# grospy/bitcoincashplus

Measured on AMD Instinct MI355X. Metric: equihash_200_9_solutions_per_sec, higher is better.
Workload: dtype uint32; 1 GPU; model=Equihash(200,9) mainnet PoW solver (BLAKE2b, K=9 collision rounds), global_batch=96, seq_len=2097152, parallelism=dp1 (nonce-space), solvers_in_flight=2, full=False, verified_solutions=0, gpu_cpu_verifier_disagreements=0, rows_dropped_all_nonces=232040, pairs_dropped_all_nonces=346057, candidates_dropped_all_nonces=0

## Files before the change

csrc/kernels/equihash_layout.h:

```cpp
#ifndef BCP_KERNELS_EQUIHASH_LAYOUT_H
#define BCP_KERNELS_EQUIHASH_LAYOUT_H

#include <cstddef>
#include <cstdint>
#include <stdexcept>

#if defined(__HIPCC__)
#define BCP_EH_HD __host__ __device__
#else
#define BCP_EH_HD
#endif

#ifndef BCP_EH_GEN_HPT
#define BCP_EH_GEN_HPT 2
#endif
#ifndef BCP_EH_GEN_NT
#define BCP_EH_GEN_NT 512
#endif
#ifndef BCP_EH_PRUNE_FROM
#define BCP_EH_PRUNE_FROM 9
#endif
#ifndef BCP_EH_MP_LATE
#define BCP_EH_MP_LATE 1
#endif
#ifndef BCP_EH_MP_LATE_FROM
#define BCP_EH_MP_LATE_FROM 8
#endif
#ifndef BCP_EH_GW
#define BCP_EH_GW 4
#endif
#ifndef BCP_EH_TABLE_PARENTS
#define BCP_EH_TABLE_PARENTS 1
#endif

namespace bcpk {

template <class C> constexpr int round_nt(int stage, bool carry);
template <class C> constexpr int round_mp(int stage, bool carry = false);
template <class C> constexpr bool round_prunes(int stage, bool carry = false);

template <int N_, int K_, int BB_, int CAP_, int NT_, int GENWG_, int NTG_, int MAXCAND_, int CAP4_ = CAP_,
          int CAP3_ = CAP_, int WGCU_ = 1, int GNT_ = 512, int GHPT_ = 2, int CAPF_ = 0, int MPX_ = 0, int GW_ = 0>
struct EhCfg {
    static constexpr int N = N_, K = K_;
    static constexpr int DB = N / (K + 1);
    static constexpr int BB = BB_;
    static constexpr int RB = DB - BB_;
    static constexpr int NB = 1 << BB_;
    static constexpr int NRESTS = 1 << RB;
    static constexpr int CAP = CAP_;
    static constexpr int CAPF = CAPF_ > 0 ? CAPF_ : CAP3_;
    static constexpr int MPX = MPX_;
    static constexpr int cap(int round) {
        return round == K_ ? CAPF : words(round - 1) >= 5 ? CAP_ : words(round - 1) == 4 ? CAP4_ : CAP3_;
// ... 32 lines not shown
    static constexpr bool tp(int stage) {
        return BCP_EH_TABLE_PARENTS && stage >= 1 && stage <= K - 2 && !round_prunes<EhCfg>(stage + 1) &&
               !round_prunes<EhCfg>(stage + 1, true) && pad(stage) >= BB;
    }
    static constexpr int ptab(int stage) {
        const int a = round_mp<EhCfg>(stage, false) * round_nt<EhCfg>(stage, false);
        const int b = GW_ > 0 ? round_mp<EhCfg>(stage, true) * round_nt<EhCfg>(stage, true) : 0;
        return a > b ? a : b;
    }
    static constexpr uint32_t tpmask(int stage) { return (1u << (pad(stage) > BB ? BB + 1 : BB)) - 1; }
    static constexpr uint32_t rmask(int stage) { return tp(stage) ? (uint32_t)NB - 1 : cp(stage) ? RMASK : 0u; }
    static constexpr int sw(int stage) {
        return stage == 0 || tp(stage) ? words(stage) : words(stage) + (cp(stage) ? 1 : 2);
    }
    static constexpr size_t ROWS = (size_t)NB * AREA;
    static constexpr bool H16 = NB > 512;
    static constexpr int HW = H16 ? NB / 2 : NB;
    static_assert(RPW * GENWG_ == INIT && RPW < 65535, "generation split");
    static_assert(RB > 0 && DB < 32, "digit geometry");
    static_assert(AREA < (1 << IB), "LDS row indices in parent words and signatures");
    static_assert(NT_ % 64 == 0 && NT_ <= 1024 && (NB <= NT_ || NB % NT_ == 0) && NB <= NTG_ && NT_ / 64 <= 64,
                  "workgroup shape");
    static_assert(words(K - 1) == 1, "final round keeps whole rows in one LDS word");
    static_assert(GW_ == 0 || (WGCU_ == 1 && RNT >= 128 && (NB <= RNT || NB % RNT == 0)), "carrying workgroup shape");
};

#ifndef BCP_EH_CAPF
#define BCP_EH_CAPF 6016
#endif
using Cfg200_9 = EhCfg<200, 9, 9, 4416, 1024, 512, 1024, 256, 4864, 5120, 1, BCP_EH_GEN_NT, BCP_EH_GEN_HPT, BCP_EH_CAPF, 0, BCP_EH_GW>;
// ... 33 lines not shown
    if (stage == C::K) return un_walk_list<C>(cap);
    const int pairs = round_mp<C>(stage, carry) * round_nt<C>(stage, carry) * 4;
    const int walk = un_walk_list<C>(cap) + pairs;
    return walk > pairs ? walk : pairs;
}
template <class C> constexpr int round_lds(int stage, bool prune, bool carry = false) {
    const int WR = C::words(stage - 1);
    const int WI = WR;
    const int cap = C::cap(stage);
    const int pruneb = prune ? cap * 4 + (C::cp(stage - 1) ? 0 : (cap * 2 + 3) / 4 * 4) : 0;
    const int hists = stage == C::K ? 0 : 2 * C::HW * 4 + (C::NB * (C::H16 ? 2 : 4) + 3) / 4 * 4;
    const int gen = carry ? 2 * C::NB * 4 + 16 * 8 : 0;
    return (cap * WI + 3) / 4 * 16 + pruneb + 4 + round_un<C>(stage, carry) + hists +
           (round_nt<C>(stage, carry) / 64 + 1) * 4 + gen;
}
template <class C> constexpr bool round_prunes(int stage, bool carry) {
    constexpr int from = C::K == 9 ? BCP_EH_PRUNE_FROM : 2;
    return (stage >= from || stage == C::K) && stage >= 2 && round_lds<C>(stage, true, carry) <= C::LDS_BUDGET;
}

template <class C> struct GenCarry {
    static constexpr int GT = C::GW > 0 ? 64 * C::GW : 64;
    static constexpr int NHASH = (C::INIT + C::IPH - 1) / C::IPH;
    static constexpr int ITERS = (C::K - 1) * C::NB;
    static constexpr int HB = ((NHASH + ITERS - 1) / ITERS + GT - 1) / GT;
    static constexpr int CH = HB * GT;
    static constexpr int RPT = HB * C::IPH;
    static constexpr int BPT = (C::NB + GT - 1) / GT;
    static_assert((long long)CH * ITERS >= NHASH, "the carrying rounds cover every hash");
};

template <class C> BCP_EH_HD inline uint64_t slot_parent(int stage, const uint32_t* slot) {
    const uint32_t* q = slot + C::words(stage);
// ... 29 lines not shown
```

csrc/kernels/equihash_solver.hip:

```cpp
#include <hip/hip_runtime.h>

#include "crypto/hashes.h"
#include "kernels/blake2b_device.h"
#include "kernels/equihash_layout.h"
#include "kernels/equihash_pow.h"
#include "kernels/gpu_api.h"
#include "kernels/hip_util.h"

#include <algorithm>
#include <cstdlib>
#include <cstring>
#include <stdexcept>
#include <utility>

#ifndef BCP_EH_XCD_MAP
#define BCP_EH_XCD_MAP 1
#endif
#ifndef BCP_EH_PF_SLICES
#define BCP_EH_PF_SLICES 3
#endif
#ifndef BCP_EH_GROUPS_DEFAULT
#define BCP_EH_GROUPS_DEFAULT(batch) ((batch) >= 48 ? (batch) / 24 : 1)
#endif

namespace bcpk {

constexpr uint32_t OOB = 0x80000000u;
typedef uint32_t u2v __attribute__((ext_vector_type(2)));
typedef uint32_t u3v __attribute__((ext_vector_type(3)));
typedef uint32_t u4v __attribute__((ext_vector_type(4)));

template <int CTRL, int ROWMASK = 0xf>
__device__ __forceinline__ uint32_t dpp0(uint32_t x) {
    return (uint32_t)__builtin_amdgcn_update_dpp(0, (int)x, CTRL, ROWMASK, 0xf, false);
// ... 308 lines not shown
#define EH_STAMP(k)                                                                                  \
    do {                                                                                             \
        if constexpr (STAMP) {                                                                       \
            if (threadIdx.x == 0) stamps[(size_t)bk * 16 + (k)] = __builtin_amdgcn_s_memtime();        \
        }                                                                                            \
    } while (0)

struct EhCarry {
    const EhBaseState* states;
    uint32_t* R0;
    uint32_t* LEAF;
    uint32_t* CTR0;
    int nonces;
};

constexpr int EH_NBAR = 10;
constexpr int EH_SCAN_BARS = 2;
template <int K> __device__ __forceinline__ void eh_bar() {
    static_assert(K >= 1 && K <= EH_NBAR, "barrier outside the bucket iteration's count");
    __syncthreads();
}
#define EH_BAR_SCAN(k) static_assert((k) >= 1 && (k) + EH_SCAN_BARS - 1 <= EH_NBAR, "scan barriers")

template <class C, int STAGE>
__device__ __forceinline__ void eh_carry_gen(const EhCarry& cy, int nbk, uint32_t* ghist, uint32_t* gbase, uint64_t* gr0p) {
    using GC = GenCarry<C>;
    constexpr int W0 = C::words(0);
    constexpr int SW = (C::N + 31) / 32 + 1;
    constexpr int SW0 = C::sw(0);
    constexpr int GT = GC::GT, HB = GC::HB;
    constexpr uint32_t OCAP = C::cap(1);
    const int gtid = (int)threadIdx.x - C::RNT;
    const int G = gridDim.x;
    auto chunk_of = [&](int b) -> int {
        const int nonce = b / C::NB, c = (STAGE - 1) * C::NB + b % C::NB;
        return (nonce < cy.nonces && (long long)c * GC::CH < GC::NHASH) ? c : -1;
    };
    auto prefix = [&](int b) {
        if (gtid == 0 && b / C::NB < cy.nonces) {
            uint64_t P[16];
            eh_hdr_round0_uniform(cy.states[b / C::NB], P);
#pragma unroll
            for (int i = 0; i < 16; ++i) gr0p[i] = P[i];
        }
    };
    constexpr int RA = 3, RB = 5, RC = 6, RD = 10;
    EhHdrHash hs[HB];
    auto start = [&](int b) {
        const int c = chunk_of(b);
        if (c < 0) return;
        const EhBaseState& bs = cy.states[b / C::NB];
        uint64_t P[16];
#pragma unroll
        for (int i = 0; i < 16; ++i) P[i] = gr0p[i];
#pragma unroll
        for (int hh = 0; hh < HB; ++hh) {
            hs[hh].begin(P, bs, (uint32_t)c * GC::CH + (uint32_t)(hh * GT + gtid));
            hs[hh].template rounds<1, RA>(bs);
        }
    };
    int it = 0;
// ... 5 lines not shown
    for (;;) {
        const int nonce = bk / C::NB;
        const int chunk = chunk_of(bk);
        const bool act = chunk >= 0;
        const EhBaseState& bs = cy.states[act ? nonce : 0];
        const int bn = xcd_bucket<C::NB>(blockIdx.x, it + 1, G, nbk);
        const bool more = bn >= 0;
        const uint32_t g0 = (uint32_t)chunk * GC::CH + (uint32_t)gtid;
        uint32_t rw[GC::RPT][W0];
        uint32_t rk[GC::RPT];
        uint32_t myb[GC::BPT];
        if (act) {
#pragma unroll
            for (int hh = 0; hh < HB; ++hh) hs[hh].template rounds<RA, RB>(bs);
        }
        eh_bar<1>();
        eh_bar<2>();
        eh_bar<3>();
        if (act) {
#pragma unroll
            for (int hh = 0; hh < HB; ++hh) hs[hh].template rounds<RB, RC>(bs);
        }
        eh_bar<4>();
        if (act) {
#pragma unroll
            for (int hh = 0; hh < HB; ++hh) hs[hh].template rounds<RC, RD>(bs);
        }
        if (more && bn / C::NB != nonce) prefix(bn);
        eh_bar<5>();
        if (act) {
#pragma unroll
            for (int hh = 0; hh < HB; ++hh) {
                hs[hh].template rounds<RD, 12>(bs);
                uint64_t h[8];
                hs[hh].finish(bs, h);
                const uint32_t g = g0 + hh * GT;
#pragma unroll
                for (int s = 0; s < C::IPH; ++s) {
                    uint32_t S[SW];
#pragma unroll
                    for (int w = 0; w < SW; ++w) {
                        uint32_t v = 0;
#pragma unroll
                        for (int t = 0; t < 4; ++t) {
                            const int k = 4 * w + t;
                            v = (v << 8) | ((k < C::NBYTES) ? digest_byte(h, s * C::NBYTES + k) : 0u);
                        }
                        S[w] = v;
                    }
                    const int q = hh * C::IPH + s;
                    const uint32_t d = S[0] >> (32 - C::BB);
#pragma unroll
                    for (int w = 0; w < W0; ++w) rw[q][w] = (S[w] << C::BB) | (S[w + 1] >> (32 - C::BB));
                    rk[q] = NIL;
                    if (g * C::IPH + s < (uint32_t)C::INIT) rk[q] = (atomicAdd(&ghist[d], 1u) << 16) | d;
                }
            }
        }
        eh_bar<6>();
        if (act) {
#pragma unroll
            for (int k = 0; k < GC::BPT; ++k) {
                const int b = gtid + k * GT;
                const uint32_t c = b < C::NB ? ghist[b] : 0u;
                myb[k] = 0;
                if (c) myb[k] = atomicAdd(&cy.CTR0[(size_t)nonce * C::NB + b], c);
            }
        }
        eh_bar<7>();
        if (act)
            for (int i = gtid; i < C::NB; i += GT) ghist[i] = 0;
        eh_bar<8>();
        if (act) {
#pragma unroll
            for (int k = 0; k < GC::BPT; ++k) {
                const int b = gtid + k * GT;
                if (b < C::NB) gbase[b] = myb[k];
            }
        }
        eh_bar<9>();
        if (act) {
            const auto rs = buf_rsrc(cy.R0 + (size_t)nonce * C::ROWS * SW0, (uint32_t)(C::ROWS * SW0 * 4));
            const auto rl = buf_rsrc(cy.LEAF + (size_t)nonce * C::ROWS, (uint32_t)(C::ROWS * 4));
#pragma unroll
            for (int q = 0; q < GC::RPT; ++q) {
                const uint32_t d = rk[q] & 0xffff;
                const uint32_t pos = gbase[d < (uint32_t)C::NB ? d : 0] + (rk[q] >> 16);
                const uint32_t slot = d * C::AREA + pos;
                const bool ok = rk[q] != NIL && pos < OCAP;
                const uint32_t li = (g0 + (q / C::IPH) * GT) * C::IPH + (q % C::IPH);
                row_store<W0>(rs, ok ? slot * (SW0 * 4) : OOB, rw[q]);
                __builtin_amdgcn_raw_buffer_store_b32(li, rl, ok ? slot * 4 : OOB, 0, 0);
            }
        }
        if (more) start(bn);
        eh_bar<EH_NBAR>();
        if (!more) break;
        bk = bn;
        ++it;
    }
}

template <class C, int STAGE, bool STAMP, bool CARRY = false>
__global__ __launch_bounds__(C::NT) __attribute__((amdgpu_waves_per_eu(C::WGCU * C::NT / 256)))
void eh_round(const uint32_t* __restrict__ Rin, const uint32_t* __restrict__ CTRin, uint32_t* __restrict__ Rout,
              uint32_t* __restrict__ CTRout, uint32_t* __restrict__ Pout, uint32_t* __restrict__ Bout,
              uint32_t* __restrict__ ncand, uint64_t* __restrict__ cand, uint64_t* __restrict__ stamps,
              uint32_t* __restrict__ pdrop, int nbk, EhCarry carry) {
    constexpr int WI = C::words(STAGE - 1);
    constexpr int WO = (STAGE < C::K) ? C::words(STAGE) : 1;
    constexpr int CAP = C::cap(STAGE);
    constexpr bool FINAL = STAGE == C::K;
    constexpr int PDW = 2 * C::K + 2;
    static_assert(!CARRY || (C::GW > 0 && !FINAL && !STAMP), "only plain collision rounds carry generation");
    constexpr bool PRUNE = round_prunes<C>(STAGE, CARRY);
    static_assert(PRUNE == round_prunes<C>(STAGE), "a carrying round prunes like the plain one");
    static_assert(round_lds<C>(STAGE, PRUNE, CARRY) <= 160 * 1024 / C::WGCU, "round LDS budget");
    constexpr int NT = round_nt<C>(STAGE, CARRY);
    static_assert(!CARRY || NT / 64 > 1, "block_exscan runs its two barriers only with more than one wave");
    constexpr int RPL = (CAP + NT - 1) / NT;
    constexpr int MP = round_mp<C>(STAGE, CARRY);
    constexpr int SWI = C::sw(STAGE - 1);
    constexpr int SWO = STAGE < C::K ? C::sw(STAGE) : 1;
    constexpr bool TPO = !FINAL && C::tp(STAGE);
    constexpr int PTW = TPO ? C::ptab(STAGE) : 1;
    static_assert(!TPO || PTW >= MP * NT, "the pair table holds every ordinal this round's emit can have (the spair bound)");
    static_assert(!(PRUNE && C::tp(STAGE - 1)), "a pruning round reads its parents from the slots");
    constexpr bool CPI = C::cp(STAGE - 1);
    constexpr uint32_t RMI = C::rmask(STAGE - 1);
    constexpr int SLI = (RPL + BCP_EH_PF_SLICES - 1) / BCP_EH_PF_SLICES;
    constexpr int BPT = (C::NB + NT - 1) / NT;
    constexpr bool FOLD = !FINAL;
    using HT = std::conditional_t<C::H16, uint16_t, uint32_t>;
    __shared__ __attribute__((aligned(16))) uint32_t rows[(CAP * WI + 3) / 4 * 4];
    __shared__ uint32_t psig[PRUNE ? CAP : 1];
    __shared__ uint16_t pdw[PRUNE && !CPI ? CAP : 1];
    __shared__ uint32_t npairs;
    __shared__ __attribute__((aligned(16))) uint8_t un[round_un<C>(STAGE, CARRY)];
    static_assert(FINAL || (sizeof(un) >= (size_t)un_walk_list<C>(CAP) + (size_t)MP * NT * 4),
                  "the union holds sidx, bend and this round's MP * NT pairs");
    __shared__ uint32_t hist_[FINAL ? 1 : C::HW], cur_[FINAL ? 1 : C::HW];
    __shared__ HT base[FINAL ? 1 : C::NB];
    __shared__ uint32_t wsum[NT / 64 + 1];
    __shared__ uint32_t ghist[CARRY ? C::NB : 1], gbase[CARRY ? C::NB : 1];
    __shared__ uint64_t gr0p[CARRY ? 16 : 1];
    uint16_t* sidx = reinterpret_cast<uint16_t*>(un);
    uint32_t* bend = reinterpret_cast<uint32_t*>(un + un_walk_bend<C>(CAP));
    uint32_t* plist = reinterpret_cast<uint32_t*>(un + un_walk_list<C>(CAP));
    uint32_t* spair = FOLD ? plist : reinterpret_cast<uint32_t*>(un);
    const int tid = threadIdx.x;
    const int G = gridDim.x;
    int it = 0;
    int bk = xcd_bucket<C::NB>(blockIdx.x, 0, G, nbk);
    if (bk < 0) return;
    if constexpr (CARRY) {
        if (__builtin_amdgcn_readfirstlane(tid >> 6) >= NT / 64) {
            eh_carry_gen<C, STAGE>(carry, nbk, ghist, gbase, gr0p);
            return;
        }
    }

    auto hget = [&](const uint32_t* h, int b) -> uint32_t {
        if constexpr (C::H16) return reinterpret_cast<const uint16_t*>(h)[b];
// ... 69 lines not shown
    if constexpr (!FINAL) {
        const auto rs_out = buf_rsrc(Rout, 0);
        const uint32_t z[SWO] = {};
        if constexpr (TPO) {
#pragma unroll
            for (int k = 0; k < BPT; ++k) __builtin_amdgcn_raw_buffer_store_b32(0u, rs_out, OOB + 256 * MP + 64 * k, 0, 0);
        }
#pragma unroll
        for (int u = 0; u < MP; ++u) {
            row_store<SWO>(rs_out, OOB + 256 * u, z);
            if constexpr (TPO) __builtin_amdgcn_raw_buffer_store_b32(0u, rs_out, OOB + 256 * u + 128, 0, 0);
        }
    }
    if constexpr (FOLD) {
        for (int k = tid; k < C::NRESTS; k += NT) bend[k] = 0;
        __syncthreads();
    }
    const int bk1 = xcd_bucket<C::NB>(blockIdx.x, 1, G, nbk);
    uint32_t fill_next = bk1 >= 0 ? CTRin[bk1] : 0u;
    const auto ctr_rs = buf_rsrc(CTRin, (uint32_t)nbk * 4);
    auto fill_of = [&](int b) -> uint32_t {
        return __builtin_amdgcn_raw_buffer_load_b32(ctr_rs, b >= 0 ? (uint32_t)b * 4 : OOB, 0, 0);
    };

    for (;;) {
        const int nonce = bk / C::NB, d = bk % C::NB;
        EH_STAMP(0);
        if (tid == 0 && fill > (uint32_t)CAP) atomicAdd(&pdrop[nonce * PDW + C::K + STAGE], fill - CAP);
        {
            const uint32_t ot = opaque_tid();
#pragma unroll
            for (int u = 0; u < RPL; ++u) {
                const uint32_t r = ot + u * NT;
// ... 1 lines not shown
                    if constexpr (WI % 2 == 0) {
#pragma unroll
                        for (int w = 0; w < WI; w += 2)
                            *reinterpret_cast<u2v*>(&rows[r * WI + w]) = u2v{nr[u][w], nr[u][w + 1]};
                    } else {
#pragma unroll
                        for (int w = 0; w < WI; ++w) rows[r * WI + w] = nr[u][w];
                    }
                    if constexpr (PRUNE) {
                        psig[r] = nr[u][WI];
                        if constexpr (!CPI) pdw[r] = (uint16_t)nr[u][WI + 1];
                    }
                    if constexpr (FOLD) {
                        const uint32_t key = nr[u][0] >> (32 - C::RB);
                        krank[u] = (key << 16) | atomicAdd(&bend[key], 1u);
                    }
                }
            }
        }
        if constexpr (!FINAL)
            for (int b = tid; b < C::HW; b += NT) hist_[b] = 0;
        if constexpr (!FOLD)
            for (int k = tid; k < C::NRESTS; k += NT) bend[k] = 0;
        if (tid == 0) npairs = 0;
        EH_STAMP(1);
        const int bn = xcd_bucket<C::NB>(blockIdx.x, it + 1, G, nbk);
        const bool more = bn >= 0;
        const uint32_t fn = more ? (uint32_t)__builtin_amdgcn_readfirstlane(fill_next) : 0u;
        const uint32_t nn = min(fn, (uint32_t)CAP);
        pf_bk = more ? bn : bk;
        pf_n = nn;
        const int bn2 = xcd_bucket<C::NB>(blockIdx.x, it + 2, G, nbk);
        issue(0, SLI);
        fill_next = fill_of(bn2);
        eh_bar<1>();
        EH_STAMP(2);

        auto key_of = [&](uint32_t i) -> uint32_t { return rows[i * WI] >> (32 - C::RB); };
        uint32_t kpairs[FOLD ? RPL : 1];
        if constexpr (FOLD) {
            EH_BAR_SCAN(2);
            block_exscan<NT, (C::NRESTS + NT - 1) / NT>(bend, C::NRESTS, wsum);
            const uint32_t ot = opaque_tid();
#pragma unroll
            for (int u = 0; u < RPL; ++u) {
                const uint32_t r = ot + u * NT;
                kpairs[u] = 0;
                if (r < n) {
                    const uint32_t key = krank[u] >> 16;
                    const uint32_t pos = bend[key] + (krank[u] & 0xffff);
                    const uint32_t e = key + 1 < (uint32_t)C::NRESTS ? bend[key + 1] : n;
                    sidx[pos] = (uint16_t)r;
                    krank[u] = pos;
                    kpairs[u] = min(e - pos - 1, 14u);
                    if (e - pos - 1 > 14u) atomicAdd(&pdrop[nonce * PDW + STAGE], e - pos - 1 - 14u);
                }
            }
        } else {
            for (uint32_t i = tid; i < n; i += NT) atomicAdd(&bend[key_of(i)], 1u);
            __syncthreads();
            block_exscan<NT, (C::NRESTS + NT - 1) / NT>(bend, C::NRESTS, wsum);
            for (uint32_t i = tid; i < n; i += NT) sidx[atomicAdd(&bend[key_of(i)], 1u)] = (uint16_t)i;
        }
        issue(SLI, 2 * SLI);
        eh_bar<4>();
        EH_STAMP(3);

        if constexpr (FINAL) {
            static_assert(WI == 1, "final-round rows are one word");
            for (uint32_t p = tid; p < n; p += NT) {
                const uint32_t i = sidx[p], ri = rows[i], e = bend[ri >> (32 - C::RB)];
                for (uint32_t q = p + 1; q < e; ++q) {
                    const uint32_t j = sidx[q];
                    if ((rows[j] ^ ri) & ~RMI) continue;
                    if constexpr (PRUNE) {
                        if (shares_parent(i, j)) continue;
                    }
                    const uint32_t c = atomicAdd(&ncand[nonce], 1u);
                    if (c < (uint32_t)C::MAXCAND) cand[(size_t)nonce * C::MAXCAND + c] = pack_tri(d, i, j);
                }
            }
            issue(2 * SLI, RPL);
        } else {
            uint32_t cnt = 0;
#pragma unroll
            for (int u = 0; u < RPL; ++u) cnt += kpairs[u];
            const uint32_t incl = wave_incl<false>(cnt);
            uint32_t wb = 0;
            if ((tid & 63) == 63) wb = atomicAdd(&npairs, incl);
            uint32_t o = __builtin_amdgcn_readlane(wb, 63) + incl - cnt;
#pragma unroll
            for (int u = 0; u < RPL; ++u) {
                if (!kpairs[u]) continue;
                const uint32_t p = krank[u];
                const uint32_t i = tid + u * NT;
                for (uint32_t q = p + 1; q <= p + kpairs[u]; ++q, ++o) {
                    if (o >= (uint32_t)(MP * NT)) continue;
                    plist[o] = ((uint32_t)sidx[q] << 16) | i;
                }
            }
            eh_bar<5>();
            EH_STAMP(7);
            const uint32_t P = npairs;
            const uint32_t Pc = min(P, (uint32_t)(MP * NT));
            if (tid == 0 && P > (uint32_t)(MP * NT)) atomicAdd(&pdrop[nonce * PDW + STAGE], P - MP * NT);
            uint32_t pv[MP], pd[MP];
#pragma unroll
            for (int u = 0; u < MP; ++u) {
                const uint32_t k = tid + u * NT;
                pv[u] = NIL;
                pd[u] = 0;
                if (k < Pc) {
                    const uint32_t pr = plist[k];
                    const uint32_t i = pr & 0xffff, j = pr >> 16;
                    uint32_t dest;
                    if (pair_keep(i, j, dest)) {
                        pv[u] = (j << 16) | i;
                        pd[u] = dest;
                        hinc(hist_, pd[u]);
                    }
                }
            }
            for (int k = tid; k < C::NRESTS; k += NT) bend[k] = 0;
            eh_bar<6>();
            EH_STAMP(4);
            uint32_t myb[BPT];
#pragma unroll
            for (int k = 0; k < BPT; ++k) {
                const int b = tid * BPT + k;
                myb[k] = 0;
                if (b < C::NB) myb[k] = atomicAdd(&CTRout[(size_t)nonce * C::NB + b], hget(hist_, b));
            }
            issue(2 * SLI, RPL);
            uint32_t start = 0;
            uint32_t np;
            EH_BAR_SCAN(7);
            if constexpr (C::H16)
                np = block_exscan<NT, BPT, uint16_t, uint16_t>(reinterpret_cast<const uint16_t*>(hist_),
                                                               reinterpret_cast<uint16_t*>(cur_), C::NB, wsum, &start);
            else
                np = block_exscan<NT, BPT>(hist_, cur_, C::NB, wsum, &start);
#pragma unroll
            for (int u = 0; u < MP; ++u)
                if (pv[u] != NIL) spair[hinc(cur_, pd[u])] = pv[u];
#pragma unroll
            for (int k = 0; k < BPT; ++k) {
                const int b = tid * BPT + k;
                const uint32_t rb = myb[k] - start;
                if (b < C::NB) {
                    base[b] = (HT)rb;
                    start += hget(hist_, b);
                }
                if constexpr (TPO) {
                    const auto rs_b = buf_rsrc(Bout + ((size_t)nonce * C::NB + d) * C::NB, C::NB * 4);
                    __builtin_amdgcn_raw_buffer_store_b32(rb, rs_b, b < C::NB ? (uint32_t)b * 4 : OOB, 0, 0);
                }
            }
            eh_bar<9>();
            EH_STAMP(5);
            constexpr uint32_t OCAP = C::cap(STAGE + 1 <= C::K ? STAGE + 1 : C::K);
            constexpr uint32_t RMO = C::rmask(STAGE);
            const auto rs_out = buf_rsrc(Rout + (size_t)nonce * C::ROWS * SWO, (uint32_t)(C::ROWS * SWO * 4));
            const auto rs_p = buf_rsrc(Pout + (TPO ? ((size_t)nonce * C::NB + d) * PTW : 0), TPO ? PTW * 4 : 0);
#pragma unroll
            for (int u = 0; u < MP; ++u) {
                const uint32_t t = tid + u * NT;
                const uint32_t pr = t < np ? spair[t] : 0u;
                const uint32_t i = pr & 0xffff, j = pr >> 16;
                uint32_t x[WI + 1], o[WO];
                lds_row_xor<WI>(rows, i, j, x);
                x[WI - 1] &= ~RMI;
                x[WI] = 0;
                const uint32_t b = (x[0] >> (32 - C::DB)) & (C::NB - 1);
// ... 6 lines not shown
#pragma unroll
                for (int w = 0; w < WO; ++w) ov[w] = o[w];
                if constexpr (TPO) {
                    ov[WO - 1] |= (uint32_t)d & RMO;
                } else if constexpr (C::cp(STAGE)) {
                    ov[WO - 1] |= (d >> C::DX) & RMO;
                    ov[WO] = cpack<C>(d, i, j);
                } else {
                    ov[WO] = (j << 16) | i;
                    ov[WO + 1] = d;
                }
                row_store<SWO>(rs_out, ok ? slot * (SWO * 4) : OOB, ov);
                if constexpr (TPO) __builtin_amdgcn_raw_buffer_store_b32(pr, rs_p, t < np ? t * 4 : OOB, 0, 0);
            }
        }
        eh_bar<EH_NBAR>();
        EH_STAMP(6);
        if (!more) break;
        bk = bn;
        ++it;
        fill = fn;
        n = nn;
    }
}


struct EhStages {
    const uint32_t* r[16];
    const uint32_t* p[16];
    const uint32_t* b[16];
};
template <class C>
// ... 153 lines not shown
    size_t bytes = 0;

    template <class C> void alloc() {
        d_states.alloc(batch);
        h_states.alloc(batch);
        static_assert(C::K <= 16, "stage arrays");
        for (int s = 0; s < C::K; ++s) d_rst[s].alloc((size_t)batch * C::ROWS * C::sw(s));
        for (int s = 0; s < C::K; ++s)
            if (C::tp(s)) {
                d_ptab[s].alloc((size_t)batch * C::NB * C::ptab(s));
                d_btab[s].alloc((size_t)batch * C::NB * C::NB);
            }
        d_ctr.alloc((size_t)C::K * batch * C::NB);
        d_leaf.alloc((size_t)batch * C::ROWS);
        d_ncand.alloc(batch);
        d_pdrop.alloc((size_t)batch * (2 * C::K + 2));
        h_pdrop.alloc((size_t)batch * (2 * C::K + 2));
        d_cand.alloc((size_t)batch * C::MAXCAND);
        d_idx.alloc((size_t)batch * C::MAXCAND * C::L);
        d_valid.alloc((size_t)batch * C::MAXCAND);
        h_ncand.alloc(batch);
        d_nout.alloc(1);
        h_nout.alloc(1);
        d_out.alloc((size_t)batch * C::MAXCAND * (C::L + 2));
        h_out.alloc((size_t)batch * C::MAXCAND * (C::L + 2));
        outq = std::min<size_t>((size_t)batch * 4 + 16, (size_t)batch * C::MAXCAND);
        h_idx.alloc((size_t)C::MAXCAND * C::L);
        h_ctr0.alloc((size_t)C::K * C::NB);
        h_ctr_all.alloc((size_t)C::K * batch * C::NB);
        d_stamps.alloc((size_t)C::K * batch * C::NB * 16);
        bytes = d_leaf.n * 4 + d_ctr.n * 4 + d_idx.n * 4;
        for (int s = 0; s < C::K; ++s) bytes += (d_rst[s].n + d_ptab[s].n + d_btab[s].n) * 4;
    }

    template <class C, int S, bool ST, bool CY> int round_grid(int nbk) {
        static int per_cu = -1;
        if (per_cu < 0) {
            int occ = 0;
            BCP_HIP_CHECK(hipOccupancyMaxActiveBlocksPerMultiprocessor(&occ, bcpk::eh_round<C, S, ST, CY>, C::NT, 0));
            per_cu = std::max(occ, 1);
        }
        return std::min(nbk, ncu * per_cu);
    }
    template <class C, int S, bool STAMP, bool CARRY> void launch_round_as(int noff, int gn, int next) {
        constexpr bool OUT = S < C::K;
        constexpr int SO = S < C::K ? S : 0;
        constexpr bool TP = OUT && C::tp(SO);
        constexpr size_t PDW = 2 * C::K + 2;
        const size_t o = (size_t)noff;
        const uint32_t* rin = d_rst[S - 1].p + o * C::ROWS * C::sw(S - 1);
        uint32_t* rout = OUT ? d_rst[SO].p + o * C::ROWS * C::sw(SO) : nullptr;
        const uint32_t* cin = d_ctr.p + ((size_t)(S - 1) * batch + o) * C::NB;
        uint32_t* cout = OUT ? d_ctr.p + ((size_t)S * batch + o) * C::NB : nullptr;
        uint32_t* pout = TP ? d_ptab[SO].p + o * C::NB * C::ptab(SO) : nullptr;
        uint32_t* bout = TP ? d_btab[SO].p + o * C::NB * C::NB : nullptr;
        uint64_t* st = STAMP ? d_stamps.p + ((size_t)(S - 1) * batch + o) * C::NB * 16 : nullptr;
        const int nbk = C::NB * gn;
        bcpk::EhCarry cy{};
        if constexpr (CARRY) {
            const size_t p = o + (size_t)gn;
            cy.states = d_states.p + p;
            cy.R0 = d_rst[0].p + p * C::ROWS * C::sw(0);
            cy.LEAF = d_leaf.p + p * C::ROWS;
// ... 161 lines not shown
        BCP_HIP_CHECK(hipSetDevice(device));
        BCP_HIP_CHECK(hipStreamSynchronize(stream));
        const int ns = inflight;
        inflight = 0;
        float ms = 0;
        BCP_HIP_CHECK(hipEventElapsedTime(&ms, ev0, ev1));
        stats.gpu_ms += ms;
        stats.nonces += ns;
        constexpr size_t K = C::K, NB = C::NB;
        stats.pair_dropped_all.resize(K + 1, 0);
        stats.stage_dropped_all.resize(K, 0);
        stats.pair_dropped_nonce.assign(ns, 0);
        stats.stage_dropped_nonce.assign(ns, 0);
        std::vector<uint64_t> pd(K + 1, 0);
        for (int nn = 0; nn < ns; ++nn) {
            const uint32_t* q = h_pdrop.p + (size_t)nn * (2 * K + 2);
            for (size_t r = 0; r <= K; ++r) {
                pd[r] += q[r];
                stats.pair_dropped_all[r] += q[r];
                stats.pair_dropped_nonce[nn] += q[r];
            }
            for (size_t s = 0; s < K; ++s) {
                stats.stage_dropped_all[s] += q[K + 1 + s];
                stats.stage_dropped_nonce[nn] += q[K + 1 + s];
            }
        }
        if (debug) stats.pair_dropped = pd;
        if (debug) {
            stats.stage_rows.assign(K, 0);
            stats.stage_dropped.assign(K, 0);
            stats.stage_maxfill.assign(K, 0);
            stats.stage_top.assign(K, {});
            stats.stage_maxfill_all.assign(K, 0);
            for (size_t s = 0; s < K; ++s)
                for (size_t x = 0; x < (size_t)ns * NB; ++x) {
                    const uint64_t fill = h_ctr_all.p[(s * batch) * NB + x];
                    stats.stage_maxfill_all[s] = std::max<uint64_t>(stats.stage_maxfill_all[s], fill);
                    if (fill > (uint64_t)C::cap(s + 1)) stats.overflow_fills.push_back((uint64_t)s << 32 | fill);
                }
// ... 315 lines not shown
```

csrc/kernels/gpu_api.h:

```cpp
#pragma once
#include <cstdint>
#include <memory>
#include <string>
#include <functional>
#include <vector>

namespace bcp {
class CBlake2b;
namespace gpu {

bool GpuAvailable();
int DeviceCount();
std::string DeviceName(int device);
void Check(int hip_status, const char* what);

struct EhBaseState {
    uint64_t h[8];
    uint64_t m[16];
    uint64_t t0;
    uint32_t g_byte;
    uint32_t outlen;
};
EhBaseState MakeEhBaseState(const CBlake2b& st);
size_t EquihashSolutionBytes(unsigned N, unsigned K);
// ... 1 lines not shown
struct EhGpuStats {
    uint64_t nonces = 0;
    uint64_t candidates = 0;
    uint64_t duplicates = 0;
    uint64_t solutions = 0;
    uint64_t dropped_rows = 0;
    uint64_t cand_dropped = 0;
    uint64_t cand_max = 0;
    double gpu_ms = 0;
    uint64_t carry_launches = 0;
    std::vector<uint64_t> stage_rows, stage_dropped, stage_maxfill;
    std::vector<std::vector<uint64_t>> stage_top;
    std::vector<uint64_t> pair_dropped;
    std::vector<uint64_t> stage_dropped_all;
    std::vector<uint64_t> pair_dropped_all;
    std::vector<uint64_t> pair_dropped_nonce;
    std::vector<uint64_t> stage_dropped_nonce;
    std::vector<uint64_t> stage_maxfill_all;
    std::vector<uint64_t> overflow_fills;
    std::vector<std::vector<uint32_t>> debug_cands;
};

struct EhPowJob {
    unsigned char prefix[108];
    unsigned char nonce_first[32];
    int count;
    unsigned char target_le[32];
};
struct EhPowHit {
    unsigned char nonce[32];
// ... 202 lines not shown
```

csrc/python/bind_gpu.cpp:

```cpp
#include "consensus/equihash.h"
#include "kernels/gpu_api.h"
#include "node/gpuverify.h"
#include "python/bind.h"
#include "node/miner.h"
#include "node/sigverify.h"
#include "secp256k1/secp256k1.h"

namespace bcp {
namespace py {

static std::vector<gpu::EhBaseState> states_from(const std::vector<CBlake2b>& sts) {
    std::vector<gpu::EhBaseState> v;
    v.reserve(sts.size());
    for (auto& s : sts) v.push_back(gpu::MakeEhBaseState(s));
    return v;
}

void bind_gpu(pyb::module_& m) {
    m.def("gpu_available", &gpu::GpuAvailable);
    m.def("gpu_device_count", &gpu::DeviceCount);
    m.def("gpu_device_name", &gpu::DeviceName);

    pyb::class_<gpu::EquihashGpuSolver>(m, "EquihashGpuSolver")
        .def(pyb::init<unsigned, unsigned, int, int>(), pyb::arg("n"), pyb::arg("k"), pyb::arg("batch") = 1,
// ... 100 lines not shown
                 d["candidates"] = st.candidates;
                 d["duplicates"] = st.duplicates;
                 d["solutions"] = st.solutions;
                 d["dropped_rows_sampled"] = st.dropped_rows;
                 d["cand_dropped"] = st.cand_dropped;
                 d["cand_max"] = st.cand_max;
                 d["gpu_ms"] = st.gpu_ms;
                 d["carry_launches"] = st.carry_launches;
                 d["stage_rows"] = st.stage_rows;
                 d["stage_dropped"] = st.stage_dropped;
                 d["stage_maxfill"] = st.stage_maxfill;
                 d["stage_top"] = st.stage_top;
                 d["pair_dropped"] = st.pair_dropped;
                 d["stage_dropped_all"] = st.stage_dropped_all;
                 d["pair_dropped_all"] = st.pair_dropped_all;
                 d["pair_dropped_nonce"] = st.pair_dropped_nonce;
                 d["stage_dropped_nonce"] = st.stage_dropped_nonce;
                 d["stage_maxfill_all"] = st.stage_maxfill_all;
                 d["overflow_fills"] = st.overflow_fills;
                 d["debug_cands"] = st.debug_cands;
                 return d;
             })
        .def("reset_stats", &gpu::EquihashGpuSolver::ResetStats)
        .def("set_debug", &gpu::EquihashGpuSolver::SetDebug)
        .def("set_stamp_mode", &gpu::EquihashGpuSolver::SetStampMode)
        .def("debug_dump", &gpu::EquihashGpuSolver::DebugDump, pyb::arg("nonce") = 0)
        .def("debug_fills", &gpu::EquihashGpuSolver::DebugFills, pyb::arg("nonce"))
        .def("phase_cycles", &gpu::EquihashGpuSolver::PhaseCycles);

    m.def(
// ... 441 lines not shown
```

Measured before the change: 10010 Sol/s.

## Replace per-bucket sort with fixed 8-slot key table plus overflow list in collision rounds

Collision rounds now record each row into a per-key table of eight 16-bit slots during the fold. Rows beyond eight per key go to a small shared overflow list. Pairs are generated from one 16-byte LDS read per key instead of an exclusive scan and a counting sort, which removes three barriers per bucket iteration and lets the carried BLAKE2b generation merge two round slices. The cost is possible pair drops when keys overflow, plus a quadratic scan of the overflow list by the first lanes. New per-stage overflow counters are exported in the stats.

```diff
diff --git a/csrc/kernels/equihash_layout.h b/csrc/kernels/equihash_layout.h
--- a/csrc/kernels/equihash_layout.h
+++ b/csrc/kernels/equihash_layout.h
@@ -33,11 +33,21 @@
 #define BCP_EH_TABLE_PARENTS 1
 #endif
 
+#ifndef BCP_EH_KEY_SLOTS
+#define BCP_EH_KEY_SLOTS 8
+#endif
+#ifndef BCP_EH_OVL
+#define BCP_EH_OVL 128
+#endif
+static_assert(BCP_EH_KEY_SLOTS == 0 || BCP_EH_KEY_SLOTS == 8, "a key's slots are one 16-byte LDS read");
+static_assert(BCP_EH_OVL >= 1 && BCP_EH_OVL <= 128, "the overflow list is walked by the first BCP_EH_OVL lanes");
+
 namespace bcpk {
 
 template <class C> constexpr int round_nt(int stage, bool carry);
 template <class C> constexpr int round_mp(int stage, bool carry = false);
 template <class C> constexpr bool round_prunes(int stage, bool carry = false);
+template <class C> constexpr bool slot_round_fits(int stage);
 
 template <int N_, int K_, int BB_, int CAP_, int NT_, int GENWG_, int NTG_, int MAXCAND_, int CAP4_ = CAP_,
           int CAP3_ = CAP_, int WGCU_ = 1, int GNT_ = 512, int GHPT_ = 2, int CAPF_ = 0, int MPX_ = 0, int GW_ = 0>
@@ -100,6 +110,12 @@
         return stage == 0 || tp(stage) ? words(stage) : words(stage) + (cp(stage) ? 1 : 2);
     }
     static constexpr size_t ROWS = (size_t)NB * AREA;
+    static constexpr int ks(int stage) {
+        return BCP_EH_KEY_SLOTS && stage >= 1 && stage < K && NRESTS >= 256 && slot_round_fits<EhCfg>(stage)
+                   ? BCP_EH_KEY_SLOTS
+                   : 0;
+    }
+    static constexpr int PDW = 2 * K + 2 + (BCP_EH_KEY_SLOTS ? 2 * K : 0);
     static constexpr bool H16 = NB > 512;
     static constexpr int HW = H16 ? NB / 2 : NB;
     static_assert(RPW * GENWG_ == INIT && RPW < 65535, "generation split");
@@ -163,9 +179,28 @@
     return (cap * WI + 3) / 4 * 16 + pruneb + 4 + round_un<C>(stage, carry) + hists +
            (round_nt<C>(stage, carry) / 64 + 1) * 4 + gen;
 }
+template <class C> constexpr int un_slot_bend() { return C::NRESTS * 8 * 2; }
+template <class C> constexpr int un_slot_ovl() { return un_slot_bend<C>() + C::NRESTS * 4; }
+template <class C> constexpr int un_slot_list() { return un_slot_ovl<C>() + BCP_EH_OVL * 4; }
+template <class C> constexpr int slot_un(int stage, bool carry = false) {
+    return un_slot_list<C>() + round_mp<C>(stage, carry) * round_nt<C>(stage, carry) * 4;
+}
+template <class C> constexpr int slot_lds(int stage, bool prune, bool carry = false) {
+    const int b = round_lds<C>(stage, prune, carry) - round_un<C>(stage, carry) + slot_un<C>(stage, carry) + 4;
+    return carry ? (b + 7) / 8 * 8 : b;
+}
+struct EhBars {
+    int n, list, filter, scan, sort;
+};
+constexpr EhBars eh_bars(bool slot) { return slot ? EhBars{7, 2, 3, 4, 6} : EhBars{10, 5, 6, 7, 9}; }
 template <class C> constexpr bool round_prunes(int stage, bool carry) {
     constexpr int from = C::K == 9 ? BCP_EH_PRUNE_FROM : 2;
     return (stage >= from || stage == C::K) && stage >= 2 && round_lds<C>(stage, true, carry) <= C::LDS_BUDGET;
+}
+
+template <class C> constexpr bool slot_round_fits(int stage) {
+    return slot_lds<C>(stage, round_prunes<C>(stage, false), false) <= C::LDS_BUDGET &&
+           (C::GW == 0 || slot_lds<C>(stage, round_prunes<C>(stage, true), true) <= C::LDS_BUDGET);
 }
 
 template <class C> struct GenCarry {
diff --git a/csrc/kernels/equihash_solver.hip b/csrc/kernels/equihash_solver.hip
--- a/csrc/kernels/equihash_solver.hip
+++ b/csrc/kernels/equihash_solver.hip
@@ -18,6 +18,15 @@
 #endif
 #ifndef BCP_EH_PF_SLICES
 #define BCP_EH_PF_SLICES 3
+#endif
+#ifndef BCP_EH_SLOT_LIST
+#define BCP_EH_SLOT_LIST 1
+#endif
+#ifndef BCP_EH_SLOT_RB
+#define BCP_EH_SLOT_RB 5
+#endif
+#ifndef BCP_EH_SLOT_RD
+#define BCP_EH_SLOT_RD 10
 #endif
 #ifndef BCP_EH_GROUPS_DEFAULT
 #define BCP_EH_GROUPS_DEFAULT(batch) ((batch) >= 48 ? (batch) / 24 : 1)
@@ -356,13 +365,12 @@
     int nonces;
 };
 
-constexpr int EH_NBAR = 10;
 constexpr int EH_SCAN_BARS = 2;
-template <int K> __device__ __forceinline__ void eh_bar() {
-    static_assert(K >= 1 && K <= EH_NBAR, "barrier outside the bucket iteration's count");
+template <int K, int NBAR> __device__ __forceinline__ void eh_bar() {
+    static_assert(K >= 1 && K <= NBAR, "barrier outside the bucket iteration's count");
     __syncthreads();
 }
-#define EH_BAR_SCAN(k) static_assert((k) >= 1 && (k) + EH_SCAN_BARS - 1 <= EH_NBAR, "scan barriers")
+#define EH_BAR_SCAN(k, nbar) static_assert((k) >= 1 && (k) + EH_SCAN_BARS - 1 <= (nbar), "scan barriers")
 
 template <class C, int STAGE>
 __device__ __forceinline__ void eh_carry_gen(const EhCarry& cy, int nbk, uint32_t* ghist, uint32_t* gbase, uint64_t* gr0p) {
@@ -386,7 +394,11 @@
             for (int i = 0; i < 16; ++i) gr0p[i] = P[i];
         }
     };
-    constexpr int RA = 3, RB = 5, RC = 6, RD = 10;
+    constexpr bool SLOT = C::ks(STAGE) > 0;
+    constexpr EhBars BAR = eh_bars(SLOT);
+    constexpr int NBAR = BAR.n;
+    constexpr int RA = 3, RB = SLOT ? BCP_EH_SLOT_RB : 5, RC = SLOT ? RB : 6, RD = SLOT ? BCP_EH_SLOT_RD : 10;
+    static_assert(RA <= RB && RB <= RC && RC <= RD && RD <= 12, "BLAKE2b slices in order");
     EhHdrHash hs[HB];
     auto start = [&](int b) {
         const int c = chunk_of(b);
@@ -422,20 +434,22 @@
 #pragma unroll
             for (int hh = 0; hh < HB; ++hh) hs[hh].template rounds<RA, RB>(bs);
         }
-        eh_bar<1>();
-        eh_bar<2>();
-        eh_bar<3>();
+        eh_bar<1, NBAR>();
+        if constexpr (!SLOT) {
+            eh_bar<2, NBAR>();
+            eh_bar<3, NBAR>();
+            if (act) {
+#pragma unroll
+                for (int hh = 0; hh < HB; ++hh) hs[hh].template rounds<RB, RC>(bs);
+            }
+            eh_bar<4, NBAR>();
+        }
         if (act) {
 #pragma unroll
-            for (int hh = 0; hh < HB; ++hh) hs[hh].template rounds<RB, RC>(bs);
-        }
-        eh_bar<4>();
-        if (act) {
-#pragma unroll
             for (int hh = 0; hh < HB; ++hh) hs[hh].template rounds<RC, RD>(bs);
         }
         if (more && bn / C::NB != nonce) prefix(bn);
-        eh_bar<5>();
+        eh_bar<BAR.list, NBAR>();
         if (act) {
 #pragma unroll
             for (int hh = 0; hh < HB; ++hh) {
@@ -465,7 +479,7 @@
                 }
             }
         }
-        eh_bar<6>();
+        eh_bar<BAR.filter, NBAR>();
         if (act) {
 #pragma unroll
             for (int k = 0; k < GC::BPT; ++k) {
@@ -475,10 +489,10 @@
                 if (c) myb[k] = atomicAdd(&cy.CTR0[(size_t)nonce * C::NB + b], c);
             }
         }
-        eh_bar<7>();
+        eh_bar<BAR.scan, NBAR>();
         if (act)
             for (int i = gtid; i < C::NB; i += GT) ghist[i] = 0;
-        eh_bar<8>();
+        eh_bar<BAR.scan + 1, NBAR>();
         if (act) {
 #pragma unroll
             for (int k = 0; k < GC::BPT; ++k) {
@@ -486,7 +500,7 @@
                 if (b < C::NB) gbase[b] = myb[k];
             }
         }
-        eh_bar<9>();
+        eh_bar<BAR.sort, NBAR>();
         if (act) {
             const auto rs = buf_rsrc(cy.R0 + (size_t)nonce * C::ROWS * SW0, (uint32_t)(C::ROWS * SW0 * 4));
             const auto rl = buf_rsrc(cy.LEAF + (size_t)nonce * C::ROWS, (uint32_t)(C::ROWS * 4));
@@ -502,7 +516,7 @@
             }
         }
         if (more) start(bn);
-        eh_bar<EH_NBAR>();
+        eh_bar<NBAR, NBAR>();
         if (!more) break;
         bk = bn;
         ++it;
@@ -519,11 +533,16 @@
     constexpr int WO = (STAGE < C::K) ? C::words(STAGE) : 1;
     constexpr int CAP = C::cap(STAGE);
     constexpr bool FINAL = STAGE == C::K;
-    constexpr int PDW = 2 * C::K + 2;
+    constexpr int PDW = C::PDW;
     static_assert(!CARRY || (C::GW > 0 && !FINAL && !STAMP), "only plain collision rounds carry generation");
     constexpr bool PRUNE = round_prunes<C>(STAGE, CARRY);
     static_assert(PRUNE == round_prunes<C>(STAGE), "a carrying round prunes like the plain one");
-    static_assert(round_lds<C>(STAGE, PRUNE, CARRY) <= 160 * 1024 / C::WGCU, "round LDS budget");
+    constexpr bool SLOT = C::ks(STAGE) > 0;
+    constexpr EhBars BAR = eh_bars(SLOT);
+    constexpr int NBAR = BAR.n;
+    constexpr int OVL = BCP_EH_OVL;
+    static_assert((SLOT ? slot_lds<C>(STAGE, PRUNE, CARRY) : round_lds<C>(STAGE, PRUNE, CARRY)) <= 160 * 1024 / C::WGCU,
+                  "round LDS budget");
     constexpr int NT = round_nt<C>(STAGE, CARRY);
     static_assert(!CARRY || NT / 64 > 1, "block_exscan runs its two barriers only with more than one wave");
     constexpr int RPL = (CAP + NT - 1) / NT;
@@ -544,17 +563,22 @@
     __shared__ uint32_t psig[PRUNE ? CAP : 1];
     __shared__ uint16_t pdw[PRUNE && !CPI ? CAP : 1];
     __shared__ uint32_t npairs;
-    __shared__ __attribute__((aligned(16))) uint8_t un[round_un<C>(STAGE, CARRY)];
-    static_assert(FINAL || (sizeof(un) >= (size_t)un_walk_list<C>(CAP) + (size_t)MP * NT * 4),
+    __shared__ uint32_t novf;
+    __shared__ __attribute__((aligned(16))) uint8_t un[SLOT ? slot_un<C>(STAGE, CARRY) : round_un<C>(STAGE, CARRY)];
+    static_assert(FINAL || SLOT || (sizeof(un) >= (size_t)un_walk_list<C>(CAP) + (size_t)MP * NT * 4),
                   "the union holds sidx, bend and this round's MP * NT pairs");
+    static_assert(!SLOT || (sizeof(un) >= (size_t)un_slot_list<C>() + (size_t)MP * NT * 4 && OVL <= NT && CAP < 0x4000),
+                  "the union holds ktab, bend, ovl and this round's MP * NT pairs; one lane per overflow entry; ranks below the flags");
     __shared__ uint32_t hist_[FINAL ? 1 : C::HW], cur_[FINAL ? 1 : C::HW];
     __shared__ HT base[FINAL ? 1 : C::NB];
     __shared__ uint32_t wsum[NT / 64 + 1];
     __shared__ uint32_t ghist[CARRY ? C::NB : 1], gbase[CARRY ? C::NB : 1];
     __shared__ uint64_t gr0p[CARRY ? 16 : 1];
     uint16_t* sidx = reinterpret_cast<uint16_t*>(un);
-    uint32_t* bend = reinterpret_cast<uint32_t*>(un + un_walk_bend<C>(CAP));
-    uint32_t* plist = reinterpret_cast<uint32_t*>(un + un_walk_list<C>(CAP));
+    uint16_t* ktab = sidx;
+    uint32_t* bend = reinterpret_cast<uint32_t*>(un + (SLOT ? un_slot_bend<C>() : un_walk_bend<C>(CAP)));
+    uint32_t* ovl = reinterpret_cast<uint32_t*>(un + un_slot_ovl<C>());
+    uint32_t* plist = reinterpret_cast<uint32_t*>(un + (SLOT ? un_slot_list<C>() : un_walk_list<C>(CAP)));
     uint32_t* spair = FOLD ? plist : reinterpret_cast<uint32_t*>(un);
     const int tid = threadIdx.x;
     const int G = gridDim.x;
@@ -654,9 +678,13 @@
     }
     if constexpr (FOLD) {
         for (int k = tid; k < C::NRESTS; k += NT) bend[k] = 0;
+        if constexpr (SLOT) {
+            if (tid == 0) novf = 0;
+        }
         __syncthreads();
     }
-    const int bk1 = xcd_bucket<C::NB>(blockIdx.x, 1, G, nbk);
+    uint32_t ovf_sum = 0, ovf_max = 0;
+    const int bk1 =xcd_bucket<C::NB>(blockIdx.x, 1, G, nbk);
     uint32_t fill_next = bk1 >= 0 ? CTRin[bk1] : 0u;
     const auto ctr_rs = buf_rsrc(CTRin, (uint32_t)nbk * 4);
     auto fill_of = [&](int b) -> uint32_t {
@@ -688,6 +716,22 @@
                     if constexpr (FOLD) {
                         const uint32_t key = nr[u][0] >> (32 - C::RB);
                         krank[u] = (key << 16) | atomicAdd(&bend[key], 1u);
+                    }
+                }
+            }
+            if constexpr (SLOT) {
+#pragma unroll
+                for (int u = 0; u < RPL; ++u) {
+                    const uint32_t r = ot + u * NT;
+                    if (r < n) {
+                        const uint32_t key = krank[u] >> 16, t = krank[u] & 0xffff;
+                        if (t < 8u) {
+                            ktab[key * 8 + t] = (uint16_t)r;
+                        } else {
+                            const uint32_t o = atomicAdd(&novf, 1u);
+                            if (o < (uint32_t)OVL) ovl[o] = (key << 16) | r;
+                            krank[u] |= o < (uint32_t)OVL ? 0x4000u : 0x8000u;
+                        }
                     }
                 }
             }
@@ -707,13 +751,18 @@
         const int bn2 = xcd_bucket<C::NB>(blockIdx.x, it + 2, G, nbk);
         issue(0, SLI);
         fill_next = fill_of(bn2);
-        eh_bar<1>();
+        eh_bar<1, NBAR>();
         EH_STAMP(2);
 
         auto key_of = [&](uint32_t i) -> uint32_t { return rows[i * WI] >> (32 - C::RB); };
         uint32_t kpairs[FOLD ? RPL : 1];
-        if constexpr (FOLD) {
-            EH_BAR_SCAN(2);
+        if constexpr (SLOT) {
+            if constexpr (STAMP) {
+                if (threadIdx.x == 0) stamps[(size_t)bk * 16 + 3] = stamps[(size_t)bk * 16 + 2];
+            }
+            issue(SLI, 2 * SLI);
+        } else if constexpr (FOLD) {
+            EH_BAR_SCAN(2, NBAR);
             block_exscan<NT, (C::NRESTS + NT - 1) / NT>(bend, C::NRESTS, wsum);
             const uint32_t ot = opaque_tid();
 #pragma unroll
@@ -736,9 +785,11 @@
             block_exscan<NT, (C::NRESTS + NT - 1) / NT>(bend, C::NRESTS, wsum);
             for (uint32_t i = tid; i < n; i += NT) sidx[atomicAdd(&bend[key_of(i)], 1u)] = (uint16_t)i;
         }
-        issue(SLI, 2 * SLI);
-        eh_bar<4>();
-        EH_STAMP(3);
+        if constexpr (!SLOT) {
+            issue(SLI, 2 * SLI);
+            eh_bar<4, NBAR>();
+            EH_STAMP(3);
+        }
 
         if constexpr (FINAL) {
             static_assert(WI == 1, "final-round rows are one word");
@@ -757,12 +808,73 @@
             issue(2 * SLI, RPL);
         } else {
             uint32_t cnt = 0;
+            uint32_t le = 0, lm = 0, ln = 0;
+            if constexpr (SLOT) {
+                const uint32_t nov = __builtin_amdgcn_readfirstlane(novf);
+                const uint32_t NO = min(nov, (uint32_t)OVL);
+                const bool full = nov > (uint32_t)OVL;
+                ovf_sum += nov;
+                ovf_max = max(ovf_max, nov);
+#pragma unroll
+                for (int u = 0; u < RPL; ++u) {
+                    kpairs[u] = 0;
+                    if (tid + u * NT < n) {
+                        const uint32_t t = krank[u] & 0x3fffu, f = krank[u] & 0xc000u;
+                        kpairs[u] = f == 0x4000u ? 0u : min(t, 8u);
+                        if (full && f) atomicAdd(&pdrop[nonce * PDW + STAGE], t - 8u);
+                    }
+                }
+                if ((uint32_t)tid < NO) {
+                    le = ovl[tid];
+                    uint32_t m = 0;
+                    for (uint32_t q = 0; q < (uint32_t)tid; ++q) m += (ovl[q] >> 16) == (le >> 16) ? 1u : 0u;
+                    lm = min(m, 6u);
+                    if (full) {
+                        if (lm) atomicSub(&pdrop[nonce * PDW + STAGE], lm);
+                    } else if (m > 6u) {
+                        atomicAdd(&pdrop[nonce * PDW + STAGE], m - 6u);
+                    }
+                    ln = 8u + lm;
+                    cnt = ln;
+                }
+            }
 #pragma unroll
             for (int u = 0; u < RPL; ++u) cnt += kpairs[u];
             const uint32_t incl = wave_incl<false>(cnt);
             uint32_t wb = 0;
             if ((tid & 63) == 63) wb = atomicAdd(&npairs, incl);
             uint32_t o = __builtin_amdgcn_readlane(wb, 63) + incl - cnt;
+            if constexpr (SLOT) {
+                auto table_pairs = [&](uint32_t key, uint32_t c, uint32_t i) {
+                    const u4v w = *reinterpret_cast<const u4v*>(&ktab[key * 8]);
+                    const uint32_t room = o < (uint32_t)(MP * NT) ? (uint32_t)(MP * NT) - o : 0u;
+                    const uint32_t ce = min(c, room);
+                    if constexpr (BCP_EH_SLOT_LIST == 1) {
+                        for (uint32_t q = 0; q < ce; ++q) {
+                            const uint32_t ww = q < 4 ? (q < 2 ? w.x : w.y) : (q < 6 ? w.z : w.w);
+                            plist[o + q] = ((q & 1) ? (ww & 0xffff0000u) : (ww << 16)) | i;
+                        }
+                    } else {
+#pragma unroll
+                        for (int q = 0; q < 8; ++q)
+                            if ((uint32_t)q < ce) plist[o + q] = ((q & 1) ? (w[q >> 1] & 0xffff0000u) : (w[q >> 1] << 16)) | i;
+                    }
+                    o += c;
+                };
+#pragma unroll
+                for (int u = 0; u < RPL; ++u)
+                    if (kpairs[u]) table_pairs(krank[u] >> 16, kpairs[u], tid + u * NT);
+                if (ln) {
+                    const uint32_t i = le & 0xffffu;
+                    table_pairs(le >> 16, 8u, i);
+                    for (uint32_t q = 0, k = 0; q < (uint32_t)tid && k < lm; ++q) {
+                        const uint32_t e = ovl[q];
+                        if ((e >> 16) != (le >> 16)) continue;
+                        if (o < (uint32_t)(MP * NT)) plist[o] = (e << 16) | i;
+                        ++o, ++k;
+                    }
+                }
+            } else {
 #pragma unroll
             for (int u = 0; u < RPL; ++u) {
                 if (!kpairs[u]) continue;
@@ -773,7 +885,8 @@
                     plist[o] = ((uint32_t)sidx[q] << 16) | i;
                 }
             }
-            eh_bar<5>();
+            }
+            eh_bar<BAR.list, NBAR>();
             EH_STAMP(7);
             const uint32_t P = npairs;
             const uint32_t Pc = min(P, (uint32_t)(MP * NT));
@@ -796,7 +909,10 @@
                 }
             }
             for (int k = tid; k < C::NRESTS; k += NT) bend[k] = 0;
-            eh_bar<6>();
+            if constexpr (SLOT) {
+                if (tid == 0) novf = 0;
+            }
+            eh_bar<BAR.filter, NBAR>();
             EH_STAMP(4);
             uint32_t myb[BPT];
 #pragma unroll
@@ -808,7 +924,7 @@
             issue(2 * SLI, RPL);
             uint32_t start = 0;
             uint32_t np;
-            EH_BAR_SCAN(7);
+            EH_BAR_SCAN(BAR.scan, NBAR);
             if constexpr (C::H16)
                 np = block_exscan<NT, BPT, uint16_t, uint16_t>(reinterpret_cast<const uint16_t*>(hist_),
                                                                reinterpret_cast<uint16_t*>(cur_), C::NB, wsum, &start);
@@ -830,7 +946,7 @@
                     __builtin_amdgcn_raw_buffer_store_b32(rb, rs_b, b < C::NB ? (uint32_t)b * 4 : OOB, 0, 0);
                 }
             }
-            eh_bar<9>();
+            eh_bar<BAR.sort, NBAR>();
             EH_STAMP(5);
             constexpr uint32_t OCAP = C::cap(STAGE + 1 <= C::K ? STAGE + 1 : C::K);
             constexpr uint32_t RMO = C::rmask(STAGE);
@@ -867,8 +983,17 @@
                 if constexpr (TPO) __builtin_amdgcn_raw_buffer_store_b32(pr, rs_p, t < np ? t * 4 : OOB, 0, 0);
             }
         }
-        eh_bar<EH_NBAR>();
+        eh_bar<NBAR, NBAR>();
         EH_STAMP(6);
+        if constexpr (SLOT) {
+            if (!more || bn / C::NB != nonce) {
+                if (tid == 0 && ovf_sum) {
+                    atomicAdd(&pdrop[nonce * PDW + 2 * C::K + 1 + STAGE], ovf_sum);
+                    atomicMax(&pdrop[nonce * PDW + 3 * C::K + 1 + STAGE], ovf_max);
+                }
+                ovf_sum = ovf_max = 0;
+            }
+        }
         if (!more) break;
         bk = bn;
         ++it;
@@ -1052,8 +1177,8 @@
         d_ctr.alloc((size_t)C::K * batch * C::NB);
         d_leaf.alloc((size_t)batch * C::ROWS);
         d_ncand.alloc(batch);
-        d_pdrop.alloc((size_t)batch * (2 * C::K + 2));
-        h_pdrop.alloc((size_t)batch * (2 * C::K + 2));
+        d_pdrop.alloc((size_t)batch * C::PDW);
+        h_pdrop.alloc((size_t)batch * C::PDW);
         d_cand.alloc((size_t)batch * C::MAXCAND);
         d_idx.alloc((size_t)batch * C::MAXCAND * C::L);
         d_valid.alloc((size_t)batch * C::MAXCAND);
@@ -1084,7 +1209,7 @@
         constexpr bool OUT = S < C::K;
         constexpr int SO = S < C::K ? S : 0;
         constexpr bool TP = OUT && C::tp(SO);
-        constexpr size_t PDW = 2 * C::K + 2;
+        constexpr size_t PDW = C::PDW;
         const size_t o = (size_t)noff;
         const uint32_t* rin = d_rst[S - 1].p + o * C::ROWS * C::sw(S - 1);
         uint32_t* rout = OUT ? d_rst[SO].p + o * C::ROWS * C::sw(SO) : nullptr;
@@ -1276,7 +1401,7 @@
         stats.stage_dropped_nonce.assign(ns, 0);
         std::vector<uint64_t> pd(K + 1, 0);
         for (int nn = 0; nn < ns; ++nn) {
-            const uint32_t* q = h_pdrop.p + (size_t)nn * (2 * K + 2);
+            const uint32_t* q = h_pdrop.p + (size_t)nn * C::PDW;
             for (size_t r = 0; r <= K; ++r) {
                 pd[r] += q[r];
                 stats.pair_dropped_all[r] += q[r];
@@ -1285,6 +1410,14 @@
             for (size_t s = 0; s < K; ++s) {
                 stats.stage_dropped_all[s] += q[K + 1 + s];
                 stats.stage_dropped_nonce[nn] += q[K + 1 + s];
+            }
+            if constexpr (C::PDW > 2 * C::K + 2) {
+                stats.overflow_rows_all.resize(K + 1, 0);
+                stats.overflow_bucket_max.resize(K + 1, 0);
+                for (size_t r = 1; r <= K; ++r) {
+                    stats.overflow_rows_all[r] += q[2 * K + 1 + r];
+                    stats.overflow_bucket_max[r] = std::max<uint64_t>(stats.overflow_bucket_max[r], q[3 * K + 1 + r]);
+                }
             }
         }
         if (debug) stats.pair_dropped = pd;
diff --git a/csrc/kernels/gpu_api.h b/csrc/kernels/gpu_api.h
--- a/csrc/kernels/gpu_api.h
+++ b/csrc/kernels/gpu_api.h
@@ -39,6 +39,7 @@
     std::vector<uint64_t> pair_dropped;
     std::vector<uint64_t> stage_dropped_all;
     std::vector<uint64_t> pair_dropped_all;
+    std::vector<uint64_t> overflow_rows_all, overflow_bucket_max;
     std::vector<uint64_t> pair_dropped_nonce;
     std::vector<uint64_t> stage_dropped_nonce;
     std::vector<uint64_t> stage_maxfill_all;
diff --git a/csrc/python/bind_gpu.cpp b/csrc/python/bind_gpu.cpp
--- a/csrc/python/bind_gpu.cpp
+++ b/csrc/python/bind_gpu.cpp
@@ -138,6 +138,8 @@
                  d["pair_dropped"] = st.pair_dropped;
                  d["stage_dropped_all"] = st.stage_dropped_all;
                  d["pair_dropped_all"] = st.pair_dropped_all;
+                 d["overflow_rows_all"] = st.overflow_rows_all;
+                 d["overflow_bucket_max"] = st.overflow_bucket_max;
                  d["pair_dropped_nonce"] = st.pair_dropped_nonce;
                  d["stage_dropped_nonce"] = st.stage_dropped_nonce;
                  d["stage_maxfill_all"] = st.stage_maxfill_all;
```

New measurement: 10360 Sol/s, median of 6. +3.5%, better.
